# yashnaray/VQ-VAE-HMM-model

Hardware: AMD Instinct MI355X
Metric: VAE_HMM train-step sequences/sec (K=3, T=200, D=5) at 1/2/4/8 MI355X (higher is better)
Workload: dtype f32; 1 GPU; cfg2: VAE_HMM train step (compute_loss+backward+Adam); global_batch=1024, per_gpu_batch=1024, seq_len=200, K=3, input_dim=5, hidden_dim=64, hidden_dim2=32, u_dim=4, trans_hidden=128, parallelism=single, hip_graph=False, step_form=fused (Adam in the backward's tail launch), eager

## Files before the change

vq-vae-hmm-model_amd/csrc/strip_bwdw.hip:

```cpp
#include "vqhmm.h"

#include <stddef.h>

#include "prof.h"
#include "strip_dev.h"

namespace vqhmm {

__device__ float g_bwdw_one = 1.0f;

namespace {
constexpr int SW_LDD = 24;
constexpr int SW_LDQ = 8;
constexpr int SW_LO = 3;
constexpr int SW_OWN = 120;
static_assert(SW_OWN % 4 == 0 && SW_LO + SW_OWN - 1 <= ST_WIN - 4, "dh1 is exact on window rows 3 .. ST_WIN - 4");

struct StripWLds {
  float RW[3 * 64 * ST_LDW];
  float RS[8 * 18 * ST_LDW];
  float RG[ST_WIN * ST_LDW];
  float RD[(ST_WIN + 2) * SB_LDE];
  float RC[4 * 256];
  float RE[ST_WIN * SW_LDQ];
  float TW[4 * 32];
};
constexpr int RW_DP = ST_WIN * ST_LDW;
constexpr int RW_DL = RW_DP + ST_WIN * SW_LDD;
static_assert(RW_DL + ST_WIN * SW_LDQ <= 3 * 64 * ST_LDW, "G2 | DP | DL fit the dec_conv2 image region");
static_assert(3 * 64 * SB_LDE <= ST_WIN * ST_LDW, "the enc_conv2 image fits the G1 region");
static_assert((ST_WIN + 2) * ST_LDW <= 8 * 18 * ST_LDW && ST_WIN * SB_LDE <= 8 * 18 * ST_LDW,
              "D1 / H2 / DH1 fit the slots region");
static_assert(sizeof(StripWLds) <= 163840, "LDS");

struct SWArgs {
  int64_t R;
  int T, ldp, D, K, H2, own;
  const float* dpar;
  const float *g2, *g1, *h1e, *q, *h2e, *xp;
  const float *img_pd, *img_d2, *img_c1, *img_e2;
  const float* gscale;
  float *dg2, *dg1, *dh1;
  int store;
  const float* cmpW;
  float* slab[6];
  float* bslab[6];
  float* cslab;
  int64_t* step_inc;
  int64_t nstrip;
  int prof_it;
};

__device__ __forceinline__ void c2_tile_n4(const float* Wc, const float* Xw, int lg4, int l16, f32x4& acc) {
  constexpr int KCP = 4, NSTEP = 3 * KCP;
  const bool live = l16 < 4;
  const int wrow = live ? l16 : 0;
  float4 av[2], bv[2];
  auto load = [&](int st, float4& a, float4& b) __attribute__((always_inline)) {
    const int tap = st / KCP, kk = st - tap * KCP;
    const int col = kk * 16 + 4 * lg4;
    a = *reinterpret_cast<const float4*>(Wc + (tap * 4 + wrow) * ST_LDW + col);
    b = *reinterpret_cast<const float4*>(Xw + (l16 + tap) * ST_LDW + col);
  };
  load(0, av[0], bv[0]);
#pragma unroll
  for (int st = 0; st < NSTEP; ++st) {
    const int cb = st & 1;
    if (st + 1 < NSTEP) load(st + 1, av[cb ^ 1], bv[cb ^ 1]);
    __builtin_amdgcn_sched_barrier(0);
    const float4 au = live ? av[cb] : make_float4(0.f, 0.f, 0.f, 0.f);
    acc = mfma16x16x4(au.x, bv[cb].x, acc);
    acc = mfma16x16x4(au.y, bv[cb].y, acc);
    acc = mfma16x16x4(au.z, bv[cb].z, acc);
    acc = mfma16x16x4(au.w, bv[cb].w, acc);
    __builtin_amdgcn_sched_barrier(0);
  }
}

typedef const __attribute__((address_space(3))) float* ldsp;
__device__ __forceinline__ ldsp to_lds(const float* p) { return (ldsp)p; }
enum { SEL_NONE = 0, SEL_A = 1, SEL_B = 2 };

template <int NT, int SEL, class FA, class FB>
__device__ __forceinline__ void wg_pass(int nstep, ldsp pa, ldsp pb, int ga, int gb, FA fa, FB fb, bool ok,
                                        f32x4 (&acc)[NT], float& bacc) {
  constexpr int NS = NT == 1 ? 4 : 2;
  float ar[NS], br[NS][NT];
  auto hide = [](ldsp& p) __attribute__((always_inline)) { asm volatile("" : "+v"(p)); };
  auto load_at = [&](int j, ldsp qa, ldsp qb) __attribute__((always_inline)) {
    ar[j % NS] = fa(qa, j);
#pragma unroll
    for (int t = 0; t < NT; ++t) br[j % NS][t] = fb(qb, j, t);
  };
  auto load = [&](int j) __attribute__((always_inline)) { load_at(j, pa, pb); };
  auto next = [&]() __attribute__((always_inline)) {
    pa += ga;
    pb += gb;
    hide(pa);
    hide(pb);
  };
  hide(pa);
  hide(pb);
  auto mma = [&](int j) __attribute__((always_inline)) {
    const float av = (SEL == SEL_A && !ok) ? 0.f : ar[j % NS];
    bacc += av;
#pragma unroll
    for (int t = 0; t < NT; ++t) acc[t] = mfma16x16x4(av, (SEL == SEL_B && !ok) ? 0.f : br[j % NS][t], acc[t]);
  };
  if constexpr (NT == 1) {
    if (nstep < 4) {
#pragma unroll
      for (int j = 0; j < 3; ++j)
        if (j < nstep) load(j);
#pragma unroll
      for (int j = 0; j < 3; ++j)
        if (j < nstep) mma(j);
      return;
    }
#pragma unroll
    for (int j = 0; j < 4; ++j) {
      load(j);
      asm volatile("" ::: "memory");
    }
    next();
    int k = 0;
    for (; k + 8 <= nstep; k += 4) {
#pragma unroll
      for (int j = 0; j < 4; ++j) {
        __builtin_amdgcn_sched_barrier(0);
        mma(j);
        __builtin_amdgcn_sched_barrier(0);
        load(j);
      }
      next();
    }
    const int rem = nstep - k - 4;
#pragma unroll
    for (int j = 0; j < 4; ++j) {
      __builtin_amdgcn_sched_barrier(0);
      mma(j);
      __builtin_amdgcn_sched_barrier(0);
      if (j < 3) load_at(j, j < rem ? pa : pa - ga, j < rem ? pb : pb - gb);
    }
#pragma unroll
    for (int j = 0; j < 3; ++j) {
      __builtin_amdgcn_sched_barrier(0);
      if (j < rem) mma(j);
    }
    return;
  }
  load(0);
  int k = 0;
  for (; k + 5 <= nstep; k += 4) {
#pragma unroll
    for (int j = 0; j < 4; ++j) {
      if (j == 3) next();
      load((j + 1) & 3);
      __builtin_amdgcn_sched_barrier(0);
      mma(j);
      __builtin_amdgcn_sched_barrier(0);
    }
  }
  const int rem = nstep - k;
#pragma unroll
  for (int j = 0; j < 4; ++j) {
    if (j < 3 && j + 1 < rem) load(j + 1);
    __builtin_amdgcn_sched_barrier(0);
    if (j < rem) mma(j);
    __builtin_amdgcn_sched_barrier(0);
  }
}


__device__ __forceinline__ float col_sum4(float v) {
  v += xor16(v);
  v += xor32(v);
  return v;
}
__device__ __forceinline__ void dec1_epi(f32x4 acc, float sc, int64_t r, int64_t R, int T, int lg4, int l16, float lsc,
                                         const f32x4 (&qdl)[3], const f32x4 (&h4)[2], const float* TWs, float* xs_dh,
                                         float* xs_dl) {
  const bool valid = row_valid(r, R, T);
  f32x4 y;
#pragma unroll
  for (int v = 0; v < 4; ++v) {
    const float yy = acc[v] * sc + 0.f;
    y[v] = valid ? yy : 0.f;
  }
  float yk[4];
#pragma unroll
  for (int k = 0; k < 4; ++k) yk[k] = __shfl(y[k], l16);
  if (r >= 0 && r < R) {
    float dq[4], sdot = 0.f;
#pragma unroll
    for (int k = 0; k < 4; ++k) {
      dq[k] = yk[k] + lsc * qdl[1][k];
      sdot = fmaf(qdl[0][k], dq[k], sdot);
    }
    float dl[4];
#pragma unroll
    for (int k = 0; k < 4; ++k) dl[k] = qdl[0][k] * (dq[k] - sdot) + lsc * qdl[2][k];
    if (lg4 == 0) *reinterpret_cast<f32x4*>(xs_dl + l16 * SW_LDQ) = f32x4{dl[0], dl[1], dl[2], dl[3]};
#pragma unroll
    for (int j = 0; j < 2; ++j) {
      const int c0 = 8 * lg4 + 4 * j;
      f32x4 o;
#pragma unroll
      for (int v = 0; v < 4; ++v) {
        float sacc = 0.f;
#pragma unroll
        for (int k = 0; k < 4; ++k) sacc = fmaf(TWs[k * 32 + c0 + v], dl[k], sacc);
        o[v] = h4[j][v] > 0.f ? sacc : 0.f;
      }
      *reinterpret_cast<f32x4*>(xs_dh + l16 * SB_LDE + c0) = o;
    }
  } else {
#pragma unroll
    for (int j = 0; j < 2; ++j) *reinterpret_cast<f32x4*>(xs_dh + l16 * SB_LDE + 8 * lg4 + 4 * j) = f32x4{0.f, 0.f, 0.f, 0.f};
    if (lg4 == 0) *reinterpret_cast<f32x4*>(xs_dl + l16 * SW_LDQ) = f32x4{0.f, 0.f, 0.f, 0.f};
  }
}
}

template <int PROF>
__global__ __launch_bounds__(512) void strip_bwdw_kernel(SWArgs a, ConvArgs f) {
  extern __shared__ float4 smem4[];
  StripWLds& sh = *reinterpret_cast<StripWLds*>(smem4);
  const int tid = threadIdx.x, lane = tid & 63, wave = tid >> 6;
  const int lg4 = lane >> 4, l16 = lane & 15;
  const int64_t R = a.R;
  const int T = a.T, own = a.own, nstep = own / 4;
  constexpr int lo = SW_LO;
  float* slot = sh.RS + wave * 18 * ST_LDW;
  if (a.step_inc && blockIdx.x == 0 && tid == 0) *a.step_inc = (*a.step_inc & 0xffffffffll) + 1;

  stamp<PROF>(0);
  if constexpr (PROF > 0) { if (tid == 0 && blockIdx.x < 256) g_prof[blockIdx.x * 16 + 13] = __builtin_amdgcn_s_memtime(); }
  const int K = a.K, D = a.D;
  float twv = 0.f;
  if (tid < 128) {
    const int k = tid >> 5, c = tid & 31;
    twv = (k < K && c < a.H2) ? f.lb_W[k * a.H2 + c] : 0.f;
  }
  {
    constexpr int NC = 3 * 4 * ST_LDW / 4;
    static_assert(NC <= 4 * 64 && sizeof(StripWLds::RC) == 4 * 1024, "one whole-chunk DMA per wave");
    const int c = min(wave, 3);
    const int i = min(c * 64 + lane, NC - 1);
    dma16(a.img_c1 + ((i / 72) * 16 * ST_LDW + (i % 72) * 4), sh.RC + c * 256);
  }
  if (tid < 128) sh.TW[tid] = twv;
  auto dma_d2 = [&]() __attribute__((always_inline)) {
    constexpr int N1 = 3 * 64 * ST_LDW / 4, C1 = N1 / 64;
    static_assert(N1 % 64 == 0 && C1 <= 56, "7 whole chunks per wave");
#pragma unroll
    for (int j = 0; j < 7; ++j) {
      const int c = min(__builtin_amdgcn_readfirstlane(wave) + 8 * j, C1 - 1);
      dma16_uncounted(a.img_d2 + c * 256, 16 * lane, sh.RW + c * 256);
    }
  };

  f32x4 accD2[6], accE2[3], accS0[1], accS1[1];
  float bD2 = 0.f, bE2 = 0.f, bS0 = 0.f, bS1 = 0.f;
#pragma unroll
  for (int t = 0; t < 6; ++t) accD2[t] = f32x4{0.f, 0.f, 0.f, 0.f};
#pragma unroll
  for (int t = 0; t < 3; ++t) accE2[t] = f32x4{0.f, 0.f, 0.f, 0.f};
  accS0[0] = accS1[0] = f32x4{0.f, 0.f, 0.f, 0.f};

  const int mlo = lo - 16 * wave, mhi = lo + own - 16 * wave;
  const int slo = max(0, mlo), shi = min(16, mhi);
  const int64_t ch = blockIdx.x;
  auto store_d2 = [&](int lg4, int l16) __attribute__((always_inline)) {
    float* out = a.slab[1] + ch * 64 * 64 * 3;
    const int ob = wave >> 1;
#pragma unroll
    for (int t = 0; t < 6; ++t) {
      const int c = ((wave & 1) * 2 + t / 3) * 16 + l16;
      *reinterpret_cast<f32x4*>(out + (c * 3 + t % 3) * 64 + ob * 16 + 4 * lg4) = accD2[t];
    }
    const float cb = col_sum4(bD2);
    if ((wave & 1) == 0 && lg4 == 0) a.bslab[1][ch * 64 + ob * 16 + l16] = cb;
  };
  auto store_s0 = [&](int lg4, int l16, int qtap, int qc, bool qok) __attribute__((always_inline)) {
    const float cb = col_sum4(bS0);
    if (wave < 4) {
      const int P = 2 * D;
#pragma unroll
      for (int v = 0; v < 4; ++v) {
        const int o = 4 * lg4 + v;
        if (o < P) a.slab[0][(ch * P + o) * 64 + wave * 16 + l16] = accS0[0][v];
      }
      if (wave == 0 && lg4 == 0 && l16 < P) a.bslab[0][ch * P + l16] = cb;
    } else {
      const int ob = wave - 4;
#pragma unroll
      for (int v = 0; v < 4; ++v)
        if (qok) a.slab[2][((ch * 64 + ob * 16 + 4 * lg4 + v) * K + qc) * 3 + qtap] = accS0[0][v];
      if (lg4 == 0) a.bslab[2][ch * 64 + ob * 16 + l16] = cb;
    }
  };
  auto store_e2 = [&](int lg4, int l16) __attribute__((always_inline)) {
    const int H2 = a.H2, ob = wave & 1;
    float* out = a.slab[4] + ch * H2 * 64 * 3;
    const int c = (wave >> 1) * 16 + l16, o0 = ob * 16 + 4 * lg4;
#pragma unroll
    for (int t = 0; t < 3; ++t) {
      float* dst = out + (c * 3 + t) * H2 + o0;
      if (H2 % 4 == 0) {
        if (o0 < H2) *reinterpret_cast<f32x4*>(dst) = accE2[t];
      } else {
#pragma unroll
        for (int v = 0; v < 4; ++v)
          if (o0 + v < H2) dst[v] = accE2[t][v];
      }
    }
    const float ce = col_sum4(bE2), cl = col_sum4(bS1);
    if (wave < 2 && lg4 == 0 && ob * 16 + l16 < H2) a.bslab[4][ch * H2 + ob * 16 + l16] = ce;
    if (wave < 2) {
#pragma unroll
      for (int v = 0; v < 4; ++v) {
        const int o = 4 * lg4 + v, c = wave * 16 + l16;
        if (o < K && c < H2) a.slab[3][(ch * K + o) * H2 + c] = accS1[0][v];
      }
      if (wave == 0 && lg4 == 0 && l16 < K) a.bslab[3][ch * K + l16] = cl;
    }
  };
  auto store_e1 = [&](int lg4, int l16, int xtap, int xc, bool xok) __attribute__((always_inline)) {
    if (wave < 4) return;
    const int ob = wave - 4;
#pragma unroll
    for (int v = 0; v < 4; ++v)
      if (xok) a.slab[5][((ch * 64 + ob * 16 + 4 * lg4 + v) * D + xc) * 3 + xtap] = accS1[0][v];
    const float cb = col_sum4(bS1);
    if (lg4 == 0) a.bslab[5][ch * 64 + ob * 16 + l16] = cb;
  };

  int it = 0;
  for (int64_t s = blockIdx.x; s < a.nstrip; s += gridDim.x) {
    const bool last = s + gridDim.x >= a.nstrip;
    int tidv = tid;
    asm volatile("" : "+v"(tidv));
    [[maybe_unused]] unsigned long long t15 = 0;
    if constexpr (PROF > 0) { if (it == a.prof_it) t15 = __builtin_amdgcn_s_memrealtime(); }
    const int z0 = tidv >> 10;
    const float psc = (a.gscale ? a.gscale : &g_bwdw_one)[z0];
    const float fsc = (f.scale ? f.scale : &g_bwdw_one)[z0];
    const float lsc = (f.lb_scale ? f.lb_scale : &g_bwdw_one)[z0];
    const int lane = tidv & 63, lg4 = lane >> 4, l16 = lane & 15;
    const int rm = ((lg4 & 1) << 1) | (lg4 >> 1);
    const int row0 = lo + rm;
    const int qtap = l16 / K, qc = l16 - qtap * K;
    const bool qok = l16 < 3 * K;
    const int xtap = l16 / D, xc = l16 - xtap * D;
    const bool xok = l16 < 3 * D;
    const int64_t s0 = s * own - SW_LO;
    const int64_t rb = s0 + 16 * wave;
    auto ld_dpar_raw = [&](int64_t r) {
      const int64_t rc = r < 0 ? 0 : (r >= R ? R - 1 : r);
      return *reinterpret_cast<const float4*>(a.dpar + rc * a.ldp + min(4 * lg4, a.ldp - 4));
    };
    auto dpar_mask = [&](int64_t r, float4 v) {
      return (r >= 0 && r < R && 4 * lg4 < a.ldp) ? v : make_float4(0.f, 0.f, 0.f, 0.f);
    };
    float4 m1[4];
    {
      float wP[4][4];
#pragma unroll
      for (int nb = 0; nb < 4; ++nb) {
        const float4 w4 = *reinterpret_cast<const float4*>(a.img_pd + (nb * 16 + l16) * ST_LDF + 4 * lg4);
        wP[nb][0] = w4.x; wP[nb][1] = w4.y; wP[nb][2] = w4.z; wP[nb][3] = w4.w;
      }
      load_mask(a.g1, rb, R, lg4, l16, m1);
      auto front = [&](const float4 x, f32x4 (&acc)[4]) {
        const float b[4] = {x.x, x.y, x.z, x.w};
#pragma unroll
        for (int nb = 0; nb < 4; ++nb) acc[nb] = f32x4{0.f, 0.f, 0.f, 0.f};
#pragma unroll
        for (int e = 0; e < 4; ++e)
#pragma unroll
          for (int nb = 0; nb < 4; ++nb) acc[nb] = mfma16x16x4(wP[nb][e], b[e], acc[nb]);
      };
      float4 mA[4], xA;
      load_mask(a.g2, rb, R, lg4, l16, mA);
      xA = ld_dpar_raw(rb + l16);
      float4 qv;
      {
        int64_t r = s0 + (tidv & (ST_WIN - 1));
        r = r < 0 ? 0 : (r >= R ? R - 1 : r);
        qv = *reinterpret_cast<const float4*>(a.q + r * 4);
      }
      asm volatile("" ::: "memory");
      if (it == a.prof_it) stamp<PROF>(10);
      f32x4 acc[4];
      front(dpar_mask(rb + l16, xA), acc);
      if constexpr (PROF > 0) {
        if (it == a.prof_it) {
          asm volatile("s_nop 0" : : "v"(acc[3][3]));
          stamp<PROF>(11);
        }
      }
      mask_epi(acc, mA, psc, rb, R, T, lg4, l16, slo, shi, a.store ? a.dg2 : nullptr, slot + ST_LDW, ST_LDW, -1,
               wave > 0 ? slot - 18 * ST_LDW + 17 * ST_LDW : nullptr, wave < 7 ? slot + 18 * ST_LDW : nullptr);
#pragma unroll
      for (int nb = 0; nb < 4; ++nb)
        *reinterpret_cast<float4*>(sh.RG + (16 * wave + l16) * ST_LDW + nb * 16 + 4 * lg4) = m1[nb];
      if (tidv < ST_WIN) *reinterpret_cast<float4*>(sh.RE + tidv * SW_LDQ) = qv;
    }
    if (it == a.prof_it) stamp<PROF>(12);
    dma_d2();
    asm volatile("s_waitcnt vmcnt(7)" ::: "memory");
    lds_barrier_dma();
    if (it == a.prof_it) stamp<PROF>(1);
    if constexpr (PROF > 0) { if (it == a.prof_it && tid == 0 && blockIdx.x < 256) g_prof[blockIdx.x * 16 + 15] = t15; }
    f32x4 mA[4];
    {
      int64_t r = rb + l16;
      r = r < 0 ? 0 : (r >= R ? R - 1 : r);
#pragma unroll
      for (int nb = 0; nb < 4; ++nb) mA[nb] = *reinterpret_cast<const f32x4*>(a.g2 + r * 64 + nb * 16 + 4 * lg4);
    }
    const float4 xA = ld_dpar_raw(rb + l16);
    {
      const float* ya = sh.RS + (wave >> 1) * 16 + l16;
      const float* xb = sh.RG + (wave & 1) * 32 + l16;
      const int a3 = (rm == 0 ? 12 : 14) * ST_LDW;
      wg_pass<6, SEL_NONE>(nstep, to_lds(ya + (row0 + 1) * ST_LDW), to_lds(xb + (row0 - 1) * ST_LDW), 18 * ST_LDW,
                           16 * ST_LDW, [&](ldsp p, int j) { return j < 3 ? p[4 * j * ST_LDW] : p[a3]; },
                           [&](ldsp p, int j, int t) { return p[(4 * j + t % 3) * ST_LDW + (t / 3) * 16]; }, true,
                           accD2, bD2);
    }
    asm volatile("s_waitcnt vmcnt(0)" ::: "memory");
    lds_barrier_dma();
    f32x4 d1[4];
    {
      f32x4 acc[4][1];
#pragma unroll
      for (int nb = 0; nb < 4; ++nb) acc[nb][0] = f32x4{0.f, 0.f, 0.f, 0.f};
      c2_mfma_tile<4, 1, 4, 3, ST_LDW, 64>(sh.RW, slot, lg4, l16, acc, true);
#pragma unroll
      for (int nb = 0; nb < 4; ++nb) d1[nb] = acc[nb][0];
      mask_epi(d1, m1, 1.0f, rb, R, T, lg4, l16, slo, shi, a.store ? a.dg1 : nullptr, nullptr, 0);
    }
    lds_barrier();
    if (it == a.prof_it) stamp<PROF>(2);
#pragma unroll
    for (int nb = 0; nb < 4; ++nb) {
      *reinterpret_cast<f32x4*>(sh.RS + (16 * wave + 1 + l16) * ST_LDW + nb * 16 + 4 * lg4) = d1[nb];
      *reinterpret_cast<f32x4*>(sh.RW + (16 * wave + l16) * ST_LDW + nb * 16 + 4 * lg4) = mA[nb];
    }
    *reinterpret_cast<float4*>(sh.RW + RW_DP + (16 * wave + l16) * SW_LDD + 4 * lg4) = dpar_mask(rb + l16, xA);
    constexpr int N2 = 3 * 64 * SB_LDE / 4, C2 = N2 / 64;
    static_assert(N2 % 64 == 0 && C2 <= 32, "4 whole chunks per wave");
    f32x4 e2v[4];
#pragma unroll
    for (int j = 0; j < 4; ++j) {
      const int c = min(wave + 8 * j, C2 - 1);
      e2v[j] = *reinterpret_cast<const f32x4*>(a.img_e2 + 4 * (c * 64 + lane));
    }
    f32x4 qdl[3], h4[2];
    {
      int64_t r = rb + l16;
      r = r < 0 ? 0 : (r >= R ? R - 1 : r);
      qdl[0] = *reinterpret_cast<const f32x4*>(f.lb_q + r * 4);
      qdl[1] = *reinterpret_cast<const f32x4*>(f.lb_dqx + r * 4);
      qdl[2] = *reinterpret_cast<const f32x4*>(f.lb_dlx + r * 4);
#pragma unroll
      for (int j = 0; j < 2; ++j) h4[j] = *reinterpret_cast<const f32x4*>(f.lb_h + r * 32 + 8 * lg4 + 4 * j);
    }
    lds_barrier_dma();
    if (it == a.prof_it) stamp<PROF>(3);
    f32x4 h2v[2];
#pragma unroll
    for (int j = 0; j < 2; ++j) {
      const int i = tidv + 512 * j, row = i >> 3;
      int64_t r = s0 + row;
      r = r < 0 ? 0 : (r >= R ? R - 1 : r);
      h2v[j] = *reinterpret_cast<const f32x4*>(a.h2e + r * 32 + (i & 7) * 4);
    }
    {
      f32x4 acc1 = f32x4{0.f, 0.f, 0.f, 0.f};
      c2_tile_n4(sh.RC, sh.RS + 16 * wave * ST_LDW, lg4, l16, acc1);
      dec1_epi(acc1, fsc, rb + l16, R, T, lg4, l16, lsc, qdl, h4, sh.TW, sh.RD + (16 * wave + 1) * SB_LDE,
               sh.RW + RW_DL + 16 * wave * SW_LDQ);
    }
    if (wave < 4) {
      const float* ya = sh.RW + RW_DP + l16;
      const float* xb = sh.RW + wave * 16 + l16;
      wg_pass<1, SEL_NONE>(nstep, to_lds(ya + row0 * SW_LDD), to_lds(xb + row0 * ST_LDW), 16 * SW_LDD, 16 * ST_LDW,
                           [&](ldsp p, int j) { return p[4 * j * SW_LDD]; },
                           [&](ldsp p, int j, int) { return p[4 * j * ST_LDW]; }, true, accS0, bS0);
    } else {
      const float* ya = sh.RS + ST_LDW + (wave - 4) * 16 + l16;
      const float* xb = sh.RE + qc;
      wg_pass<1, SEL_B>(nstep, to_lds(ya + row0 * ST_LDW), to_lds(xb + (row0 - 1 + (qok ? qtap : 0)) * SW_LDQ),
                        16 * ST_LDW, 16 * SW_LDQ, [&](ldsp p, int j) { return p[4 * j * ST_LDW]; },
                        [&](ldsp p, int j, int) { return p[4 * j * SW_LDQ]; }, qok, accS0, bS0);
    }
    float4 m2[4];
    load_mask(a.h1e, rb, R, lg4, l16, m2);
#pragma unroll
    for (int j = 0; j < 4; ++j) *reinterpret_cast<f32x4*>(sh.RG + min(wave + 8 * j, C2 - 1) * 256 + 4 * lane) = e2v[j];
    lds_barrier_dma();
    if (it == a.prof_it) stamp<PROF>(4);
#pragma unroll
    for (int nb = 0; nb < 4; ++nb)
      *reinterpret_cast<float4*>(sh.RW + (16 * wave + l16) * ST_LDW + nb * 16 + 4 * lg4) = m2[nb];
#pragma unroll
    for (int j = 0; j < 2; ++j) {
      const int i = tidv + 512 * j;
      *reinterpret_cast<f32x4*>(sh.RS + (i >> 3) * SB_LDE + (i & 7) * 4) = h2v[j];
    }
    lds_barrier();
    if (it == a.prof_it) stamp<PROF>(5);
    const int xsh = ld4(D) == 8 ? 1 : 0;
    float4 xv = make_float4(0.f, 0.f, 0.f, 0.f);
    if (tidv < (ST_WIN << xsh)) {
      int64_t r = s0 + (tidv >> xsh);
      r = r < 0 ? 0 : (r >= R ? R - 1 : r);
      xv = *reinterpret_cast<const float4*>(a.xp + (r << (2 + xsh)) + (tidv & xsh) * 4);
    }
    f32x4 y[4];
    {
      f32x4 acc[4][1];
#pragma unroll
      for (int nb = 0; nb < 4; ++nb) acc[nb][0] = f32x4{0.f, 0.f, 0.f, 0.f};
      c2_mfma_tile<4, 1, 2, 3, SB_LDE, 64>(sh.RG, sh.RD + 16 * wave * SB_LDE, lg4, l16, acc, true);
#pragma unroll
      for (int nb = 0; nb < 4; ++nb) y[nb] = acc[nb][0];
      mask_epi(y, m2, 1.0f, rb, R, T, lg4, l16, slo, shi, a.store ? a.dh1 : nullptr, nullptr, 0);
    }
    {
      const float* ya = sh.RD + SB_LDE + (wave & 1) * 16 + l16;
      const float* xb = sh.RW + (wave >> 1) * 16 + l16;
      wg_pass<3, SEL_NONE>(nstep, to_lds(ya + row0 * SB_LDE), to_lds(xb + (row0 - 1) * ST_LDW), 16 * SB_LDE, 16 * ST_LDW,
                           [&](ldsp p, int j) { return p[4 * j * SB_LDE]; },
                           [&](ldsp p, int j, int t) { return p[(4 * j + t) * ST_LDW]; }, true, accE2, bE2);
    }
    if (wave < 2) {
      const float* ya = sh.RW + RW_DL + min(l16, 3);
      const float* xb = sh.RS + wave * 16 + l16;
      wg_pass<1, SEL_A>(nstep, to_lds(ya + row0 * SW_LDQ), to_lds(xb + row0 * SB_LDE), 16 * SW_LDQ, 16 * SB_LDE,
                        [&](ldsp p, int j) { return p[4 * j * SW_LDQ]; },
                        [&](ldsp p, int j, int) { return p[4 * j * SB_LDE]; }, l16 < K, accS1, bS1);
    }
    lds_barrier();
    if (it == a.prof_it) stamp<PROF>(6);
#pragma unroll
    for (int nb = 0; nb < 4; ++nb)
      *reinterpret_cast<f32x4*>(sh.RS + (16 * wave + l16) * ST_LDW + nb * 16 + 4 * lg4) = y[nb];
    if (tidv < (ST_WIN << xsh)) *reinterpret_cast<float4*>(sh.RD + (tidv >> xsh) * SW_LDQ + (tidv & xsh) * 4) = xv;
    if (last) {
#pragma unroll
      for (int j = 0; j < 6; ++j) {
        const int c = __builtin_amdgcn_readfirstlane(wave) + 8 * j;
        dma16_uncounted(a.cmpW + c * 256, 16 * lane, sh.RW + c * 256);
      }
      for (int i = tidv; i < 1536; i += 512) sh.RG[i] = 0.f;
    }
    lds_barrier_dma();
    if (wave >= 4) {
      const float* ya = sh.RS + (wave - 4) * 16 + l16;
      const float* xb = sh.RD + xc;
      wg_pass<1, SEL_B>(nstep, to_lds(ya + row0 * ST_LDW), to_lds(xb + (row0 - 1 + (xok ? xtap : 0)) * SW_LDQ),
                        16 * ST_LDW, 16 * SW_LDQ, [&](ldsp p, int j) { return p[4 * j * ST_LDW]; },
                        [&](ldsp p, int j, int) { return p[4 * j * SW_LDQ]; }, xok, accS1, bS1);
    }
    lds_barrier_dma();
    if (it == a.prof_it) stamp<PROF>(7);
    ++it;
  }

  {
    const int qtap = l16 / K, qc = l16 - qtap * K;
    const bool qok = l16 < 3 * K;
    const int xtap = l16 / D, xc = l16 - xtap * D;
    const bool xok = l16 < 3 * D;
    store_d2(lg4, l16);
    store_s0(lg4, l16, qtap, qc, qok);
    store_e2(lg4, l16);
    store_e1(lg4, l16, xtap, xc, xok);
  }
  {
    const int qtap = l16 / K, qc = l16 - qtap * K;
    const bool qok = l16 < 3 * K;
    const int h = tid & 63, g = tid >> 6;
    float* cbuf = sh.RG;
    float* part = sh.RG + 1536;
    const float* Wl = sh.RW;
    if (wave >= 4) {
      const int ob = wave - 4;
#pragma unroll
      for (int v = 0; v < 4; ++v)
        if (qok) cbuf[((ob * 16 + 4 * lg4 + v) * 3 + qtap) * 8 + qc] = accS0[0][v];
    }
    asm volatile("s_waitcnt vmcnt(0)" ::: "memory");
    lds_barrier();
    float acc[8];
#pragma unroll
    for (int k = 0; k < 8; ++k) acc[k] = 0.f;
#pragma unroll
    for (int i = 0; i < 8; ++i)
#pragma unroll
      for (int tap = 0; tap < 3; ++tap) {
        const float4* c4 = reinterpret_cast<const float4*>(cbuf + ((g + 8 * i) * 3 + tap) * 8);
        const float4 l = c4[0], hh = c4[1];
        const float cv[8] = {l.x, l.y, l.z, l.w, hh.x, hh.y, hh.z, hh.w};
        const float wv = Wl[((g + 8 * i) * 64 + h) * 3 + tap];
#pragma unroll
        for (int k = 0; k < 8; ++k) acc[k] = fmaf(cv[k], wv, acc[k]);
      }
#pragma unroll
    for (int k = 0; k < 8; ++k) part[(g * 8 + k) * 64 + h] = acc[k];
    lds_barrier();
    if (tid < K * 64) {
      const int k = tid >> 6;
      float v = 0.f;
#pragma unroll
      for (int gg = 0; gg < 8; ++gg) v += part[(gg * 8 + k) * 64 + h];
      a.cslab[ch * K * 64 + tid] = v;
    }
  }
  if constexpr (PROF > 0) {
    __syncthreads();
    stamp<PROF>(8);
    if (threadIdx.x == 0 && blockIdx.x < 256) {
      g_prof[blockIdx.x * 16 + 14] = __builtin_amdgcn_s_memtime();
      g_prof[blockIdx.x * 16 + 9] = (unsigned long long)it;
    }
  }
}

int bwdw_prof_copy(uint64_t* out, int64_t n) { return prof_copy(out, n); }

static int prof_on() {
  static const int v = prof_env("VQHMM_STRIP_PROF");
  return v;
}

bool strip_bwdw_supported(const ConvArgs& pd, const ConvArgs& d2, const ConvArgs& f, const ConvArgs& e2, int D) {
  return strip_bwd_supported(pd, d2, f, e2) && D >= 1 && 3 * D <= 16 && pd.Kc == 2 * D && f.N >= 1 && f.N <= 4 &&
         3 * f.N <= 16;
}

int strip_bwdw_own(int64_t R) {
  const int64_t rounds = cdiv(R, 256ll * SW_OWN);
  const int64_t own = cdiv(cdiv(R, 256 * rounds), 4) * 4;
  return (int)(own < 4 ? 4 : own > SW_OWN ? SW_OWN : own);
}

int strip_bwdw_grid(int64_t R) {
  const int64_t n = cdiv(R, strip_bwdw_own(R));
  return (int)(n < 256 ? (n > 0 ? n : 1) : 256);
}

int launch_strip_bwdw(const ConvArgs& pd, const ConvArgs& d2, const ConvArgs& f, const ConvArgs& e2,
                      const StripWgradArgs& w, hipStream_t s) {
  if (!strip_bwdw_supported(pd, d2, f, e2, w.D) || w.H2 != f.lb_C || w.K != f.N) return VQHMM_EUNSUPPORTED;
  SWArgs a{};
  a.R = pd.R; a.T = pd.T; a.ldp = ld4(pd.Kc); a.D = w.D; a.K = w.K; a.H2 = w.H2;
  a.own = strip_bwdw_own(pd.R);
  a.dpar = pd.src; a.g2 = pd.aux; a.g1 = d2.aux; a.h1e = e2.aux; a.q = f.lb_q; a.h2e = f.lb_h; a.xp = w.x;
  a.img_pd = pd.Wimg; a.img_d2 = d2.Wimg; a.img_c1 = f.Wimg; a.img_e2 = e2.Wimg;
  a.gscale = pd.scale;
  a.store = w.store;
  a.dg2 = pd.out; a.dg1 = d2.out; a.dh1 = e2.out;
  a.cmpW = w.cmpW;
  for (int i = 0; i < 6; ++i) {
    a.slab[i] = w.slab[i];
    a.bslab[i] = w.bslab[i];
  }
  a.cslab = w.cslab;
  a.step_inc = w.step_inc;
  a.nstrip = cdiv(pd.R, a.own);
  {
    static const int pit = prof_env("VQHMM_STRIP_PROF_IT");
    a.prof_it = pit;
  }
  const unsigned grid = (unsigned)strip_bwdw_grid(pd.R);
  if (prof_on()) strip_bwdw_kernel<1><<<grid, 512, sizeof(StripWLds), s>>>(a, f);
  else strip_bwdw_kernel<0><<<grid, 512, sizeof(StripWLds), s>>>(a, f);
  VQHMM_LAUNCH_CHECK();
  return VQHMM_OK;
}

}
```

Measured before the change: 2.712 million sequences/s.

## Hoist loop-invariant lane math, use scalar-base global loads, fuse S1 pass into E2

Lane-derived indices (row0, qtap, xtap, xsh and similar) move out of the strip loop. Global loads now use a scalar per-strip base plus a 32-bit clamped lane offset instead of per-lane 64-bit clamped addresses, which cuts VALU address arithmetic. The h1e mask load is issued earlier so its latency overlaps the preceding MFMA passes. Waves 0-1 run a new fused wg_pass_x that interleaves the S1 accumulation with the E2 pass, so S1 no longer needs a second serial pass; this raises register pressure and removes the tidv>>10 dependency on z0 by fixing z0 to 0.

```diff
diff --git a/vq-vae-hmm-model_amd/csrc/strip_bwdw.hip b/vq-vae-hmm-model_amd/csrc/strip_bwdw.hip
--- a/vq-vae-hmm-model_amd/csrc/strip_bwdw.hip
+++ b/vq-vae-hmm-model_amd/csrc/strip_bwdw.hip
@@ -79,6 +79,10 @@
 
 typedef const __attribute__((address_space(3))) float* ldsp;
 __device__ __forceinline__ ldsp to_lds(const float* p) { return (ldsp)p; }
+template <class V>
+__device__ __forceinline__ V ld_so(const float* sbase, int off, int imm = 0) {
+  return *reinterpret_cast<const V*>(reinterpret_cast<const char*>(sbase) + (unsigned)off + imm);
+}
 enum { SEL_NONE = 0, SEL_A = 1, SEL_B = 2 };
 
 template <int NT, int SEL, class FA, class FB>
@@ -149,6 +153,64 @@
     }
     return;
   }
+  load(0);
+  int k = 0;
+  for (; k + 5 <= nstep; k += 4) {
+#pragma unroll
+    for (int j = 0; j < 4; ++j) {
+      if (j == 3) next();
+      load((j + 1) & 3);
+      __builtin_amdgcn_sched_barrier(0);
+      mma(j);
+      __builtin_amdgcn_sched_barrier(0);
+    }
+  }
+  const int rem = nstep - k;
+#pragma unroll
+  for (int j = 0; j < 4; ++j) {
+    if (j < 3 && j + 1 < rem) load(j + 1);
+    __builtin_amdgcn_sched_barrier(0);
+    if (j < rem) mma(j);
+    __builtin_amdgcn_sched_barrier(0);
+  }
+}
+
+template <int NT, class FA, class FB, class FC, class FD>
+__device__ __forceinline__ void wg_pass_x(int nstep, ldsp pa, ldsp pb, int ga, int gb, FA fa, FB fb, f32x4 (&acc)[NT],
+                                          float& bacc, ldsp pc, ldsp pd, int gc, int gd, FC fc, FD fd, bool okx,
+                                          f32x4& accx, float& baccx) {
+  float ar[2], br[2][NT], cr[2], dr[2];
+  auto hide = [](ldsp& p) __attribute__((always_inline)) { asm volatile("" : "+v"(p)); };
+  auto load = [&](int j) __attribute__((always_inline)) {
+    ar[j % 2] = fa(pa, j);
+#pragma unroll
+    for (int t = 0; t < NT; ++t) br[j % 2][t] = fb(pb, j, t);
+    cr[j % 2] = fc(pc, j);
+    dr[j % 2] = fd(pd, j);
+  };
+  auto next = [&]() __attribute__((always_inline)) {
+    pa += ga;
+    pb += gb;
+    pc += gc;
+    pd += gd;
+    hide(pa);
+    hide(pb);
+    hide(pc);
+    hide(pd);
+  };
+  hide(pa);
+  hide(pb);
+  hide(pc);
+  hide(pd);
+  auto mma = [&](int j) __attribute__((always_inline)) {
+    const float av = ar[j % 2];
+    bacc += av;
+#pragma unroll
+    for (int t = 0; t < NT; ++t) acc[t] = mfma16x16x4(av, br[j % 2][t], acc[t]);
+    const float cv = okx ? cr[j % 2] : 0.f;
+    baccx += cv;
+    accx = mfma16x16x4(cv, dr[j % 2], accx);
+  };
   load(0);
   int k = 0;
   for (; k + 5 <= nstep; k += 4) {
@@ -336,42 +398,49 @@
     if (lg4 == 0) a.bslab[5][ch * 64 + ob * 16 + l16] = cb;
   };
 
+  const int rm = ((lg4 & 1) << 1) | (lg4 >> 1);
+  const int row0 = lo + rm;
+  const int qtap = l16 / K, qc = l16 - qtap * K;
+  const bool qok = l16 < 3 * K;
+  const int xtap = l16 / D, xc = l16 - xtap * D;
+  const bool xok = l16 < 3 * D;
+  const int wrow = 16 * wave + l16;
+  const int xsh = ld4(D) == 8 ? 1 : 0;
+
   int it = 0;
   for (int64_t s = blockIdx.x; s < a.nstrip; s += gridDim.x) {
     const bool last = s + gridDim.x >= a.nstrip;
-    int tidv = tid;
-    asm volatile("" : "+v"(tidv));
     [[maybe_unused]] unsigned long long t15 = 0;
     if constexpr (PROF > 0) { if (it == a.prof_it) t15 = __builtin_amdgcn_s_memrealtime(); }
-    const int z0 = tidv >> 10;
+    int z0 = 0;
+    asm volatile("" : "+v"(z0));
     const float psc = (a.gscale ? a.gscale : &g_bwdw_one)[z0];
     const float fsc = (f.scale ? f.scale : &g_bwdw_one)[z0];
     const float lsc = (f.lb_scale ? f.lb_scale : &g_bwdw_one)[z0];
-    const int lane = tidv & 63, lg4 = lane >> 4, l16 = lane & 15;
-    const int rm = ((lg4 & 1) << 1) | (lg4 >> 1);
-    const int row0 = lo + rm;
-    const int qtap = l16 / K, qc = l16 - qtap * K;
-    const bool qok = l16 < 3 * K;
-    const int xtap = l16 / D, xc = l16 - xtap * D;
-    const bool xok = l16 < 3 * D;
     const int64_t s0 = s * own - SW_LO;
     const int64_t rb = s0 + 16 * wave;
-    auto ld_dpar_raw = [&](int64_t r) {
-      const int64_t rc = r < 0 ? 0 : (r >= R ? R - 1 : r);
-      return *reinterpret_cast<const float4*>(a.dpar + rc * a.ldp + min(4 * lg4, a.ldp - 4));
+    const int wlo = s0 < 0 ? (int)-s0 : 0;
+    const int whi = R - 1 - s0 < ST_WIN - 1 ? (int)(R - 1 - s0) : ST_WIN - 1;
+    auto clampw = [&](int w) { return min(max(w, wlo), whi); };
+    const int cw = clampw(wrow);
+    const bool inr = cw == wrow;
+    const int off64 = cw * 256 + 16 * lg4;
+    auto ldw = [&](const float* m, float4 (&aux)[4]) __attribute__((always_inline)) {
+      const float* sb = m + s0 * 64;
+#pragma unroll
+      for (int nb = 0; nb < 4; ++nb) aux[nb] = ld_so<float4>(sb, off64, 64 * nb);
     };
-    auto dpar_mask = [&](int64_t r, float4 v) {
-      return (r >= 0 && r < R && 4 * lg4 < a.ldp) ? v : make_float4(0.f, 0.f, 0.f, 0.f);
-    };
+    auto ld_dpar_raw = [&]() { return ld_so<float4>(a.dpar + s0 * a.ldp, 4 * (cw * a.ldp + min(4 * lg4, a.ldp - 4))); };
+    auto dpar_mask = [&](float4 v) { return (inr && 4 * lg4 < a.ldp) ? v : make_float4(0.f, 0.f, 0.f, 0.f); };
     float4 m1[4];
     {
       float wP[4][4];
 #pragma unroll
       for (int nb = 0; nb < 4; ++nb) {
-        const float4 w4 = *reinterpret_cast<const float4*>(a.img_pd + (nb * 16 + l16) * ST_LDF + 4 * lg4);
+        const float4 w4 = ld_so<float4>(a.img_pd, 4 * (l16 * ST_LDF + 4 * lg4), nb * 16 * ST_LDF * 4);
         wP[nb][0] = w4.x; wP[nb][1] = w4.y; wP[nb][2] = w4.z; wP[nb][3] = w4.w;
       }
-      load_mask(a.g1, rb, R, lg4, l16, m1);
+      ldw(a.g1, m1);
       auto front = [&](const float4 x, f32x4 (&acc)[4]) {
         const float b[4] = {x.x, x.y, x.z, x.w};
 #pragma unroll
@@ -382,18 +451,13 @@
           for (int nb = 0; nb < 4; ++nb) acc[nb] = mfma16x16x4(wP[nb][e], b[e], acc[nb]);
       };
       float4 mA[4], xA;
-      load_mask(a.g2, rb, R, lg4, l16, mA);
-      xA = ld_dpar_raw(rb + l16);
-      float4 qv;
-      {
-        int64_t r = s0 + (tidv & (ST_WIN - 1));
-        r = r < 0 ? 0 : (r >= R ? R - 1 : r);
-        qv = *reinterpret_cast<const float4*>(a.q + r * 4);
-      }
+      ldw(a.g2, mA);
+      xA = ld_dpar_raw();
+      const float4 qv = ld_so<float4>(a.q + s0 * 4, 16 * clampw(tid & (ST_WIN - 1)));
       asm volatile("" ::: "memory");
       if (it == a.prof_it) stamp<PROF>(10);
       f32x4 acc[4];
-      front(dpar_mask(rb + l16, xA), acc);
+      front(dpar_mask(xA), acc);
       if constexpr (PROF > 0) {
         if (it == a.prof_it) {
           asm volatile("s_nop 0" : : "v"(acc[3][3]));
@@ -405,7 +469,7 @@
 #pragma unroll
       for (int nb = 0; nb < 4; ++nb)
         *reinterpret_cast<float4*>(sh.RG + (16 * wave + l16) * ST_LDW + nb * 16 + 4 * lg4) = m1[nb];
-      if (tidv < ST_WIN) *reinterpret_cast<float4*>(sh.RE + tidv * SW_LDQ) = qv;
+      if (tid < ST_WIN) *reinterpret_cast<float4*>(sh.RE + tid * SW_LDQ) = qv;
     }
     if (it == a.prof_it) stamp<PROF>(12);
     dma_d2();
@@ -414,13 +478,9 @@
     if (it == a.prof_it) stamp<PROF>(1);
     if constexpr (PROF > 0) { if (it == a.prof_it && tid == 0 && blockIdx.x < 256) g_prof[blockIdx.x * 16 + 15] = t15; }
     f32x4 mA[4];
-    {
-      int64_t r = rb + l16;
-      r = r < 0 ? 0 : (r >= R ? R - 1 : r);
-#pragma unroll
-      for (int nb = 0; nb < 4; ++nb) mA[nb] = *reinterpret_cast<const f32x4*>(a.g2 + r * 64 + nb * 16 + 4 * lg4);
-    }
-    const float4 xA = ld_dpar_raw(rb + l16);
+#pragma unroll
+    for (int nb = 0; nb < 4; ++nb) mA[nb] = ld_so<f32x4>(a.g2 + s0 * 64, off64, 64 * nb);
+    const float4 xA = ld_dpar_raw();
     {
       const float* ya = sh.RS + (wave >> 1) * 16 + l16;
       const float* xb = sh.RG + (wave & 1) * 32 + l16;
@@ -449,35 +509,32 @@
       *reinterpret_cast<f32x4*>(sh.RS + (16 * wave + 1 + l16) * ST_LDW + nb * 16 + 4 * lg4) = d1[nb];
       *reinterpret_cast<f32x4*>(sh.RW + (16 * wave + l16) * ST_LDW + nb * 16 + 4 * lg4) = mA[nb];
     }
-    *reinterpret_cast<float4*>(sh.RW + RW_DP + (16 * wave + l16) * SW_LDD + 4 * lg4) = dpar_mask(rb + l16, xA);
+    *reinterpret_cast<float4*>(sh.RW + RW_DP + (16 * wave + l16) * SW_LDD + 4 * lg4) = dpar_mask(xA);
     constexpr int N2 = 3 * 64 * SB_LDE / 4, C2 = N2 / 64;
     static_assert(N2 % 64 == 0 && C2 <= 32, "4 whole chunks per wave");
     f32x4 e2v[4];
 #pragma unroll
     for (int j = 0; j < 4; ++j) {
-      const int c = min(wave + 8 * j, C2 - 1);
-      e2v[j] = *reinterpret_cast<const f32x4*>(a.img_e2 + 4 * (c * 64 + lane));
+      const int c = min(__builtin_amdgcn_readfirstlane(wave) + 8 * j, C2 - 1);
+      e2v[j] = ld_so<f32x4>(a.img_e2 + c * 256, 16 * lane);
     }
     f32x4 qdl[3], h4[2];
-    {
-      int64_t r = rb + l16;
-      r = r < 0 ? 0 : (r >= R ? R - 1 : r);
-      qdl[0] = *reinterpret_cast<const f32x4*>(f.lb_q + r * 4);
-      qdl[1] = *reinterpret_cast<const f32x4*>(f.lb_dqx + r * 4);
-      qdl[2] = *reinterpret_cast<const f32x4*>(f.lb_dlx + r * 4);
-#pragma unroll
-      for (int j = 0; j < 2; ++j) h4[j] = *reinterpret_cast<const f32x4*>(f.lb_h + r * 32 + 8 * lg4 + 4 * j);
-    }
+    qdl[0] = ld_so<f32x4>(f.lb_q + s0 * 4, 16 * cw);
+    qdl[1] = ld_so<f32x4>(f.lb_dqx + s0 * 4, 16 * cw);
+    qdl[2] = ld_so<f32x4>(f.lb_dlx + s0 * 4, 16 * cw);
+#pragma unroll
+    for (int j = 0; j < 2; ++j) h4[j] = ld_so<f32x4>(f.lb_h + s0 * 32, 128 * cw + 32 * lg4, 16 * j);
     lds_barrier_dma();
     if (it == a.prof_it) stamp<PROF>(3);
     f32x4 h2v[2];
 #pragma unroll
     for (int j = 0; j < 2; ++j) {
-      const int i = tidv + 512 * j, row = i >> 3;
-      int64_t r = s0 + row;
-      r = r < 0 ? 0 : (r >= R ? R - 1 : r);
-      h2v[j] = *reinterpret_cast<const f32x4*>(a.h2e + r * 32 + (i & 7) * 4);
-    }
+      const int i = tid + 512 * j;
+      h2v[j] = ld_so<f32x4>(a.h2e + s0 * 32, 128 * clampw(i >> 3) + 16 * (i & 7));
+    }
+    float4 m2[4];
+    ldw(a.h1e, m2);
+    asm volatile("" ::: "memory");
     {
       f32x4 acc1 = f32x4{0.f, 0.f, 0.f, 0.f};
       c2_tile_n4(sh.RC, sh.RS + 16 * wave * ST_LDW, lg4, l16, acc1);
@@ -497,8 +554,6 @@
                         16 * ST_LDW, 16 * SW_LDQ, [&](ldsp p, int j) { return p[4 * j * ST_LDW]; },
                         [&](ldsp p, int j, int) { return p[4 * j * SW_LDQ]; }, qok, accS0, bS0);
     }
-    float4 m2[4];
-    load_mask(a.h1e, rb, R, lg4, l16, m2);
 #pragma unroll
     for (int j = 0; j < 4; ++j) *reinterpret_cast<f32x4*>(sh.RG + min(wave + 8 * j, C2 - 1) * 256 + 4 * lane) = e2v[j];
     lds_barrier_dma();
@@ -508,18 +563,12 @@
       *reinterpret_cast<float4*>(sh.RW + (16 * wave + l16) * ST_LDW + nb * 16 + 4 * lg4) = m2[nb];
 #pragma unroll
     for (int j = 0; j < 2; ++j) {
-      const int i = tidv + 512 * j;
+      const int i = tid + 512 * j;
       *reinterpret_cast<f32x4*>(sh.RS + (i >> 3) * SB_LDE + (i & 7) * 4) = h2v[j];
     }
     lds_barrier();
     if (it == a.prof_it) stamp<PROF>(5);
-    const int xsh = ld4(D) == 8 ? 1 : 0;
-    float4 xv = make_float4(0.f, 0.f, 0.f, 0.f);
-    if (tidv < (ST_WIN << xsh)) {
-      int64_t r = s0 + (tidv >> xsh);
-      r = r < 0 ? 0 : (r >= R ? R - 1 : r);
-      xv = *reinterpret_cast<const float4*>(a.xp + (r << (2 + xsh)) + (tidv & xsh) * 4);
-    }
+    const float4 xv = ld_so<float4>(a.xp + (s0 << (2 + xsh)), (clampw(tid >> xsh) << (4 + xsh)) + 16 * (tid & xsh));
     f32x4 y[4];
     {
       f32x4 acc[4][1];
@@ -533,30 +582,33 @@
     {
       const float* ya = sh.RD + SB_LDE + (wave & 1) * 16 + l16;
       const float* xb = sh.RW + (wave >> 1) * 16 + l16;
-      wg_pass<3, SEL_NONE>(nstep, to_lds(ya + row0 * SB_LDE), to_lds(xb + (row0 - 1) * ST_LDW), 16 * SB_LDE, 16 * ST_LDW,
-                           [&](ldsp p, int j) { return p[4 * j * SB_LDE]; },
-                           [&](ldsp p, int j, int t) { return p[(4 * j + t) * ST_LDW]; }, true, accE2, bE2);
-    }
-    if (wave < 2) {
-      const float* ya = sh.RW + RW_DL + min(l16, 3);
-      const float* xb = sh.RS + wave * 16 + l16;
-      wg_pass<1, SEL_A>(nstep, to_lds(ya + row0 * SW_LDQ), to_lds(xb + row0 * SB_LDE), 16 * SW_LDQ, 16 * SB_LDE,
-                        [&](ldsp p, int j) { return p[4 * j * SW_LDQ]; },
-                        [&](ldsp p, int j, int) { return p[4 * j * SB_LDE]; }, l16 < K, accS1, bS1);
+      auto fa = [&](ldsp p, int j) { return p[4 * j * SB_LDE]; };
+      auto fb = [&](ldsp p, int j, int t) { return p[(4 * j + t) * ST_LDW]; };
+      if (wave < 2) {
+        const float* yc = sh.RW + RW_DL + min(l16, 3);
+        const float* xd = sh.RS + wave * 16 + l16;
+        wg_pass_x<3>(nstep, to_lds(ya + row0 * SB_LDE), to_lds(xb + (row0 - 1) * ST_LDW), 16 * SB_LDE, 16 * ST_LDW, fa, fb,
+                     accE2, bE2, to_lds(yc + row0 * SW_LDQ), to_lds(xd + row0 * SB_LDE), 16 * SW_LDQ, 16 * SB_LDE,
+                     [&](ldsp p, int j) { return p[4 * j * SW_LDQ]; }, [&](ldsp p, int j) { return p[4 * j * SB_LDE]; },
+                     l16 < K, accS1[0], bS1);
+      } else {
+        wg_pass<3, SEL_NONE>(nstep, to_lds(ya + row0 * SB_LDE), to_lds(xb + (row0 - 1) * ST_LDW), 16 * SB_LDE,
+                             16 * ST_LDW, fa, fb, true, accE2, bE2);
+      }
     }
     lds_barrier();
     if (it == a.prof_it) stamp<PROF>(6);
 #pragma unroll
     for (int nb = 0; nb < 4; ++nb)
       *reinterpret_cast<f32x4*>(sh.RS + (16 * wave + l16) * ST_LDW + nb * 16 + 4 * lg4) = y[nb];
-    if (tidv < (ST_WIN << xsh)) *reinterpret_cast<float4*>(sh.RD + (tidv >> xsh) * SW_LDQ + (tidv & xsh) * 4) = xv;
+    if (tid < (ST_WIN << xsh)) *reinterpret_cast<float4*>(sh.RD + (tid >> xsh) * SW_LDQ + (tid & xsh) * 4) = xv;
     if (last) {
 #pragma unroll
       for (int j = 0; j < 6; ++j) {
         const int c = __builtin_amdgcn_readfirstlane(wave) + 8 * j;
         dma16_uncounted(a.cmpW + c * 256, 16 * lane, sh.RW + c * 256);
       }
-      for (int i = tidv; i < 1536; i += 512) sh.RG[i] = 0.f;
+      for (int i = tid; i < 1536; i += 512) sh.RG[i] = 0.f;
     }
     lds_barrier_dma();
     if (wave >= 4) {
```

Measured after the change: 2.762 million sequences/s, median of 6. 1.9% higher.
